# RokLenarcic/AhoCorasick

Measured on AMD Instinct MI355X. Metric: haystack MB/s (UTF-16 bytes scanned per second, records delivered in reference order), higher is better.
Workload: dtype u16; 1 GPU; BASELINE config 2: AhoCorasickMap, 10k keywords (len 4-12, a-z), 2^29 UTF-16 units (1 GiB at 29); keywords=10000, states=58221, classes=27, table=dense u16, lds_states=2408, units_per_gpu=536870912, matches_per_gpu=1332068, matches_total=1332068, record_bytes=12, parallelism=single, reserve_cus=0

## Files before the change

ahocorasick_amd/csrc/acgpu_kernels.hip:

```cpp
#include <hip/hip_runtime.h>

#include <algorithm>
#include <type_traits>
#include <utility>

#include "acgpu_device.h"
#include "acgpu_forms.h"

namespace acgpu {

#ifndef ACGPU_SCAN_MINBLOCKS
#define ACGPU_SCAN_MINBLOCKS 1
#endif
#ifndef ACGPU_DFA_CHAINS
#define ACGPU_DFA_CHAINS 2
#endif
constexpr int kScanBlock = 1024;
constexpr int kQueueCap = 128;
constexpr int kQueueFlush = kQueueCap - kWave;

int scan_block_threads() { return kScanBlock; }
size_t scan_queue_bytes(int block_threads) { return (size_t)(block_threads / kWave) * kQueueCap * sizeof(ScratchRec); }

struct WaveQueue {
// ... 765 lines not shown
    return hipGetLastError();
}


struct TokenTables {
    const uint16_t *kw_units;
    const uint32_t *kw_off;
    uint32_t n_kw;
    const uint16_t *swapcase;
    const uint16_t *script_units;
    uint32_t script_off[7];
    uint16_t seps[6];
};
__device__ __forceinline__ uint64_t synth_draw(uint64_t seed, uint64_t idx) {
    uint64_t x = seed + (idx + 1) * 0x9E3779B97F4A7C15ull;
    uint64_t z = (x ^ (x >> 30)) * 0xBF58476D1CE4E5B9ull;
    z = (z ^ (z >> 27)) * 0x94D049BB133111EBull;
    return z ^ (z >> 31);
}
__device__ __forceinline__ uint32_t synth_bounded(uint64_t z, uint32_t k) { return (uint32_t)(((z >> 32) * (uint64_t)k) >> 32); }

__global__ __launch_bounds__(256) void k_token_lengths(TokenTables T, uint64_t seed, uint32_t n_tokens, uint32_t *len) {
    const uint32_t t = blockIdx.x * blockDim.x + threadIdx.x;
    if (t >= n_tokens) return;
    const uint64_t d0 = (uint64_t)t * 32;
    uint32_t wl;
    if (synth_bounded(synth_draw(seed, d0), 2) == 0 && T.n_kw) {
        const uint32_t wi = synth_bounded(synth_draw(seed, d0 + 1), T.n_kw);
        wl = T.kw_off[wi + 1] - T.kw_off[wi];
    } else {
        wl = 2 + synth_bounded(synth_draw(seed, d0 + 2), 11);
    }
    len[t] = wl + 1 + synth_bounded(synth_draw(seed, d0 + 28), 3);
}

__global__ __launch_bounds__(256) void k_token_fill(TokenTables T, uint64_t seed, uint32_t n_tokens, const uint64_t *start, uint16_t *dst,
                                                    uint64_t n_units) {
    const uint32_t t = blockIdx.x * blockDim.x + threadIdx.x;
    if (t >= n_tokens) return;
    uint64_t at = start[t];
    if (at >= n_units) return;
    const uint64_t d0 = (uint64_t)t * 32;
    auto put = [&](uint32_t u) {
        if (at < n_units) dst[at] = (uint16_t)u;
        ++at;
    };
    if (synth_bounded(synth_draw(seed, d0), 2) == 0 && T.n_kw) {
        const uint32_t wi = synth_bounded(synth_draw(seed, d0 + 1), T.n_kw);
        const uint32_t a = T.kw_off[wi], wl = T.kw_off[wi + 1] - a;
        for (uint32_t i = 0; i < wl; ++i) {
            uint32_t u = T.kw_units[a + i];
            if (T.swapcase && i < 24 && synth_bounded(synth_draw(seed, d0 + 2 + i), 2)) u = T.swapcase[u];
            put(u);
        }
    } else {
        const uint32_t sc = synth_bounded(synth_draw(seed, d0 + 1), 6);
        const uint32_t wl = 2 + synth_bounded(synth_draw(seed, d0 + 2), 11);
        const uint32_t a = T.script_off[sc], tl = T.script_off[sc + 1] - a;
        for (uint32_t i = 0; i < wl; ++i) put(T.script_units[a + synth_bounded(synth_draw(seed, d0 + 3 + i), tl)]);
    }
    const uint32_t ns = 1 + synth_bounded(synth_draw(seed, d0 + 28), 3);
    for (uint32_t i = 0; i < ns; ++i) put(T.seps[synth_bounded(synth_draw(seed, d0 + 29 + i), 6)]);
}

hipError_t launch_token_stream(uint16_t *d_dst, uint64_t n_units, uint64_t seed, const uint16_t *d_kw_units, const uint32_t *d_kw_off,
                               uint32_t n_kw, const uint16_t *d_swapcase, const uint16_t *d_script_units, const uint32_t *script_off,
                               const uint16_t *seps, uint32_t n_tokens, uint32_t *d_len, uint64_t *d_start, uint64_t *d_tmp,
                               hipStream_t stream) {
    TokenTables T;
    T.kw_units = d_kw_units; T.kw_off = d_kw_off; T.n_kw = n_kw; T.swapcase = d_swapcase; T.script_units = d_script_units;
    for (int i = 0; i < 7; ++i) T.script_off[i] = script_off[i];
    for (int i = 0; i < 6; ++i) T.seps[i] = seps[i];
    const dim3 grid((n_tokens + 255) / 256), block(256);
    hipLaunchKernelGGL(k_token_lengths, grid, block, 0, stream, T, seed, n_tokens, d_len);
    hipError_t e = hipGetLastError();
    if (e != hipSuccess) return e;
    e = launch_exclusive_scan(d_len, n_tokens, d_start, d_tmp, stream);
    if (e != hipSuccess) return e;
    hipLaunchKernelGGL(k_token_fill, grid, block, 0, stream, T, seed, n_tokens, d_start, d_dst, n_units);
    return hipGetLastError();
}

__global__ __launch_bounds__(1024) void k_stream_probe(const uint4 *__restrict__ p, uint64_t n_tiles, unsigned *sink) {
    const uint32_t lane = threadIdx.x & 63u;
    const uint64_t wave = (uint64_t)blockIdx.x * (blockDim.x / 64) + threadIdx.x / 64;
    const uint64_t n_waves = (uint64_t)gridDim.x * (blockDim.x / 64);
    const uint64_t per_wave = (n_tiles + n_waves - 1) / n_waves;
    const uint64_t t0 = wave * per_wave, t1 = t0 + per_wave < n_tiles ? t0 + per_wave : n_tiles;
    if (t0 >= t1) return;
    uint32_t x = 0;
    uint4 cur[4], nxt[4];
    const uint4 *b = p + t0 * 256 + lane * 4;
#pragma unroll
    for (int u = 0; u < 4; ++u) nxt[u] = b[u];
    for (uint64_t t = t0; t < t1; ++t) {
#pragma unroll
        for (int u = 0; u < 4; ++u) cur[u] = nxt[u];
        const uint4 *nb = p + (t + 1 < t1 ? t + 1 : t) * 256 + lane * 4;
#pragma unroll
        for (int u = 0; u < 4; ++u) nxt[u] = nb[u];
#pragma unroll
        for (int u = 0; u < 4; ++u) x ^= cur[u].x ^ cur[u].y ^ cur[u].z ^ cur[u].w;
    }
    if (x == 0x12345678u) sink[0] = x;
}

__global__ __launch_bounds__(256) void k_stream_probe_best(const uint4 *__restrict__ p, uint64_t n_groups, unsigned *sink) {
    const uint32_t lane = threadIdx.x & 63u;
    const uint64_t wave = (uint64_t)blockIdx.x * (blockDim.x / 64) + threadIdx.x / 64;
    const uint64_t n_waves = (uint64_t)gridDim.x * (blockDim.x / 64);
    uint32_t x = 0;
    for (uint64_t g = wave; g < n_groups; g += n_waves) {
        uint4 buf[4][2];
#pragma unroll
        for (int d = 0; d < 4; ++d) {
            const uint4 *b = p + (g * 4 + d) * 128;
            buf[d][0] = b[lane * 2];
            buf[d][1] = b[lane * 2 + 1];
        }
#pragma unroll
        for (int d = 0; d < 4; ++d) x ^= buf[d][0].x ^ buf[d][0].y ^ buf[d][0].z ^ buf[d][0].w ^ buf[d][1].x ^ buf[d][1].y ^ buf[d][1].z ^ buf[d][1].w;
    }
    if (x == 0x12345678u) sink[0] = x;
}

hipError_t launch_stream_probe(const void *d_buf, uint64_t n_bytes, int n_cu, unsigned *d_sink, int pattern, hipStream_t stream) {
    if (pattern == 1) {
        const uint64_t n_groups = n_bytes / 8192;
        if (n_groups == 0) return hipErrorInvalidValue;
        hipLaunchKernelGGL(k_stream_probe_best, dim3(n_cu * 8), dim3(256), 0, stream, reinterpret_cast<const uint4 *>(d_buf), n_groups, d_sink);
        return hipGetLastError();
    }
    const uint64_t n_tiles = n_bytes / 4096;
    if (n_tiles == 0) return hipErrorInvalidValue;
    hipLaunchKernelGGL(k_stream_probe, dim3(n_cu), dim3(1024), 0, stream, reinterpret_cast<const uint4 *>(d_buf), n_tiles, d_sink);
    return hipGetLastError();
}

}
```

ahocorasick_amd/csrc/acgpu_tile.hip:

```cpp
#include <hip/hip_runtime.h>

#include <utility>

#include "acgpu_tile_common.h"

namespace acgpu {

int tile_block_threads() { return kTileBlock; }
uint32_t tile_reserve_slots() { return kReserve; }
uint32_t tile_group_units() { return kPrefetch * kTileUnits; }

#ifndef ACGPU_FILTER_WORDS
#define ACGPU_FILTER_WORDS 22016
#endif
constexpr int kFilterWordsMax = ACGPU_FILTER_WORDS;

static_assert(kVerifyBatches * kWave + 128 <= kL2Cap, "the queue holds what a drain leaves plus a tile's survivors (-DACGPU_NB=4 hangs)");
constexpr int kBigFresh = 704;
static_assert(kBigFresh * 2 * (kTileBlock / kWave) <= kL2Words * 4, "the lists of the large second level live where the Bloom words did");

struct __attribute__((packed, aligned(2))) Units8 {
    uint32_t d[4];
};

struct Vec16 {
    unsigned long long lo, hi;
};
__device__ __forceinline__ Vec16 stream_load(const uint16_t *hay, uint32_t unit) {
    const unsigned char *p = reinterpret_cast<const unsigned char *>(hay) + (size_t)(unit * 2u);
    typedef unsigned long long v2ul __attribute__((ext_vector_type(2)));
#ifdef ACGPU_STREAM_NT
    const v2ul v = __builtin_nontemporal_load(reinterpret_cast<const v2ul *>(p));
#else
    const v2ul v = *reinterpret_cast<const v2ul *>(p);
#endif
    return Vec16{v.x, v.y};
}

template <bool RANGE>
__device__ __forceinline__ uint32_t tile_class_t(const DevTables &T, uint32_t unit) {
    if (RANGE) return min(unit - T.cls_base, T.cls_span);
    if (T.hashk && T.fold_range) {
        if (unit & T.fr_himask) return T.tile_lut[unit];
        return min(min(min(unit - T.fr_base, unit - T.fr_base2), min(unit - T.fr_base3, unit - T.fr_base4)), T.fr_span);
    }
    return T.tile_lut[unit];
}

__device__ __forceinline__ uint32_t rchild(const DevTables &T, uint32_t id, uint32_t unit, uint32_t cls) {
    if (T.rdense) return T.rtab[id * T.filt_n + cls];
    const uint32_t u = T.cs ? unit : (uint32_t)T.lower[unit];
    const uint32_t r = hashed_goto(T.rhkeys, T.rhvals, T.rhmask, id, u);
    return r == ~0u ? 0u : r;
}

template <bool RANGE>
__device__ __forceinline__ uint32_t walk_step(const DevTables &T, uint32_t ref, uint32_t unit) {
    const uint32_t cls = tile_class_t<RANGE>(T, unit);
    const uint32_t hint = (ref >> kRefHintShift) & kRefHintMask;
    if (hint != 0 && hint - 1 != cls) return 0;
    return rchild(T, ref & kRefIdMask, unit, cls);
}

template <int K, bool RANGE, bool HASHK = false, bool QI = false, bool SHORTS = true>
__device__ __forceinline__ void verify_multi(TileCtx &c, uint32_t head, uint32_t n_cand) {
    constexpr int NB = kVerifyBatches;
    const DevTables &T = *c.Tp;
    const TileLaunch &L = *c.Lp;
    const uint16_t *hay = L.d_hay;
    const uint32_t lane = lane_id();
    bool act[NB];
    uint32_t e[NB], ref[NB], ref0[NB], child0[NB], left_unit[NB], d[NB], m[NB], one_len[NB], one_node[NB], info[NB], lcls[NB];
    Units8 win[NB];
#pragma unroll
    for (int b = 0; b < NB; ++b) {
        const uint32_t q = b * kWave + lane;
        act[b] = q < n_cand;
        if (QI) {
            e[b] = act[b] ? c.pos_base + (uint32_t)c.pos16[head + q] + 1 : 8;
            info[b] = act[b] ? c.cand[head + q] : 0u;
        } else {
            e[b] = act[b] ? c.cand[head + q] + 1 : 8;
            info[b] = 0;
        }
        m[b] = 0; one_len[b] = 0; one_node[b] = 0; d[b] = K; left_unit[b] = 0;
    }
    uint32_t kidx[NB];
    bool need_win = true;
    if (QI) {
        bool unknown = false;
#pragma unroll
        for (int b = 0; b < NB; ++b) unknown |= act[b] && !(info[b] & kQiKnown);
        need_win = __any(unknown);
    }
#ifdef ACGPU_TIMING
    unsigned long long vt0 = clock64();
#define VT_MARK(i) { asm volatile("s_waitcnt vmcnt(0)" ::: "memory"); const unsigned long long t_ = clock64(); c.vt[i] += t_ - vt0; vt0 = t_; }
#else
#define VT_MARK(i)
#endif
#pragma unroll
    for (int b = 0; b < NB; ++b) {
        if (!need_win) {
            win[b] = Units8{{0, 0, 0, 0}};
        } else if (e[b] >= 8) {
            if (ACGPU_DBG(L, 8u)) win[b] = Units8{{e[b], e[b] * 3u, e[b] * 5u, e[b] * 7u}};
            else win[b] = *reinterpret_cast<const Units8 *>(hay + e[b] - 8);
        } else {
            win[b] = Units8{{0, 0, 0, 0}};
#pragma unroll
            for (int j = 0; j < 8; ++j) {
                if (e[b] + j >= 8) win[b].d[j >> 1] |= (uint32_t)hay[e[b] + j - 8] << (16 * (j & 1));
            }
        }
    }
    VT_MARK(0)
#pragma unroll
    for (int b = 0; b < NB; ++b) {
        uint32_t idx = 0;
// ... 334 lines not shown
__global__ __launch_bounds__(kTileBlock) void k_ac_tile(DevTables T, TileLaunch L) {
    static_assert(!BIG || L2, "the large second level is a form of the L2 kernel");
#ifdef ACGPU_TIMING
    const unsigned long long tm_entry = clock64();
    unsigned long long tm_startup = 0;
#endif
    const bool has_short = SHORTS && T.has_short != 0;
    __shared__ __attribute__((aligned(16))) uint32_t rows32[SPLIT ? kFilterWordsSplit : (L2 ? kFilterWordsL2 : kFilterWordsMax)];
    extern __shared__ __attribute__((aligned(16))) unsigned char smem[];
    __shared__ uint32_t wg_words[kFtWords];
    const bool FT = !SPLIT && L.fused_tail != 0;
    const unsigned char *rows8 = reinterpret_cast<const unsigned char *>(rows32);
    uint32_t *cand_all = reinterpret_cast<uint32_t *>(smem);
    constexpr uint32_t kRowsPer = (sizeof(rows32) / 16 + kTileBlock - 1) / kTileBlock;
    constexpr uint32_t kBloomPer = (L2 && !BIG) ? (kL2Words / 4 + kTileBlock - 1) / kTileBlock : 0u;
    const uint32_t n4 = T.filt_words / 4;
    const uint4 *src4 = reinterpret_cast<const uint4 *>(T.filt_bits);
    uint4 tab[kRowsPer + kBloomPer];
#pragma unroll
    for (uint32_t q = 0; q < kRowsPer; ++q) {
        const uint32_t i = threadIdx.x + q * blockDim.x;
        tab[q] = make_uint4(0u, 0u, 0u, 0u);
        if (i < n4) tab[q] = src4[i];
    }
#pragma unroll
    for (uint32_t q = 0; q < kBloomPer; ++q) {
        const uint32_t i = threadIdx.x + q * blockDim.x;
        tab[kRowsPer + q] = reinterpret_cast<const uint4 *>(T.l2_bloom)[min(i, (uint32_t)kL2Words / 4 - 1)];
    }
    if (FT) {
        if (threadIdx.x == 0) ft_take_number(L, wg_words);
        __syncthreads();
    }
    const uint32_t pg_off = (T.filt_words * 4u + 15u) & ~15u;
    const bool cls_lds = !RANGE && !PK && T.cls_pages != nullptr && (uint64_t)pg_off + T.cls_pages_bytes <= sizeof(rows32) && !ACGPU_DBG(L, 1u << 15);
    const unsigned char *pg8 = rows8 + pg_off;
    constexpr int D2 = K + 2 < 6 ? K + 2 : 6;
    constexpr int kAcVec = L2 ? kL2Vec : acgpu::kAcVec;
    constexpr int kAcLaneUnits = 8 * kAcVec;
    constexpr int kAcTileUnits = kWave * kAcLaneUnits;
    constexpr int kAcTiles = kPrefetch / kAcVec;
    static_assert(kAcTiles >= 1 && kAcLaneUnits <= 32, "tile geometry");
    constexpr int kAcCandCap = kAcTileUnits + kVerifyBatches * kWave;
    constexpr uint32_t kQueueCap = L2 ? kL2Cap : kAcCandCap;
    const uint32_t wave_in_block = __builtin_amdgcn_readfirstlane(threadIdx.x / kWave);
    constexpr int kWavesPerBlock = kTileBlock / kWave;
    uint16_t *pos16_all = reinterpret_cast<uint16_t *>(smem + kWavesPerBlock * kL2Cap * 4);
    unsigned char *tb = smem + kWavesPerBlock * kL2Cap * 6 + wave_in_block * kTbBytes;
    uint16_t *fresh = reinterpret_cast<uint16_t *>(smem + kWavesPerBlock * (kL2Cap * 6 + kTbBytes)) + wave_in_block * kL2Fresh;
    uint32_t *bloom = reinterpret_cast<uint32_t *>(smem + (kTileBlock / kWave) * kL2WaveBytes);
    uint16_t *bigl = reinterpret_cast<uint16_t *>(bloom) + wave_in_block * kBigFresh;
    static_assert(kL2Words % 4 == 0, "Bloom words are copied 16 bytes at a time");

    const uint32_t lane = lane_id();
    const uint32_t wg = FT ? __builtin_amdgcn_readfirstlane(wg_words[0]) : blockIdx.x;
    const uint32_t wave_global = wg * (kTileBlock / kWave) + wave_in_block;
    TileCtx c{&T, &L, SPLIT ? L.d_cands + (size_t)wave_global * L.cands_per_wave : cand_all + wave_in_block * kQueueCap, 0, 0, 0u, 0};
    c.wg = wg;
    if (L2) c.pos16 = pos16_all + wave_in_block * kL2Cap;
    uint32_t lane0 = 0;
    const uint32_t slice_base = SPLIT ? wave_global * L.cands_per_wave : 0u;
    uint32_t region_first = 0;

    constexpr uint32_t ROWB = WIDE ? 8 : 4;
    const uint32_t n = T.filt_n;
    uint32_t nK1s = ROWB;
#pragma unroll
    for (int i = 0; i < K - 1; ++i) nK1s *= n;
    const int neg_nK1s = -(int)nK1s;
    constexpr int NP = L2 ? D2 / 2 : K / 2;

    const uint32_t first_region = wave_global * L.regions_per_wave;
    const bool has_work = first_region < L.n_regions;
    const uint32_t last_region = min(first_region + L.regions_per_wave, L.n_regions);
    const uint32_t base8 = L.own_begin & ~7u;
    const uint32_t R = L.region_units;
    const uint32_t span_begin = max(L.own_begin, base8 + first_region * R);
    uint32_t span_end = base8 + last_region * R;
    if (span_end > L.own_end || last_region == L.n_regions) span_end = L.own_end;
    const uint32_t nfull = L.n_units & ~7u;
    const uint32_t hi = min(span_end, nfull);
    const uint32_t last_vec = nfull >= 8 ? nfull - 8 : 0;
    const uint16_t *hay = L.d_hay;

    uint32_t wave_total = 0;
    uint32_t region = first_region;
    uint32_t boundary = base8 + (region + 1) * R;
    uint32_t rb = span_begin;
    uint32_t re = min(span_end, boundary);
    c.pos_base = boundary - R;
    uint32_t tile = base8 + first_region * R;

    bool vec_todo = has_work && tile < hi;
    bool tail_todo = has_work && span_end > nfull;
    uint32_t d0 = 0;
    uint32_t prio_turn = 0;
    bool mid = false;
    uint32_t carry[4] = {0, 0, 0, 0};
    Vec16 nxt[kAcTiles][kAcVec], grp[kAcTiles][kAcVec];
#pragma unroll
    for (int d = 0; d < kAcTiles; ++d)
#pragma unroll
        for (int u = 0; u < kAcVec; ++u) nxt[d][u] = grp[d][u] = Vec16{0ull, 0ull};
    if (vec_todo) {
        if (K > 1 && tile >= 8) {
            const uint4 p = *reinterpret_cast<const uint4 *>(hay + tile - 8);
            carry[0] = p.x; carry[1] = p.y; carry[2] = p.z; carry[3] = p.w;
        }
#pragma unroll
        for (int d = 0; d < kAcTiles; ++d)
#pragma unroll
            for (int u = 0; u < kAcVec; ++u)
                nxt[d][u] = stream_load(hay, min(tile + d * kAcTileUnits + lane * kAcLaneUnits + u * 8, last_vec));
    }
    {
        uint4 *dst4 = reinterpret_cast<uint4 *>(rows32);
#pragma unroll
        for (uint32_t q = 0; q < kRowsPer; ++q) {
            const uint32_t i = threadIdx.x + q * blockDim.x;
            if (i < n4) dst4[i] = tab[q];
        }
        for (uint32_t i = threadIdx.x + kRowsPer * blockDim.x; i < n4; i += blockDim.x) dst4[i] = src4[i];
        for (uint32_t i = n4 * 4 + threadIdx.x; i < T.filt_words; i += blockDim.x) rows32[i] = T.filt_bits[i];
#pragma unroll
        for (uint32_t q = 0; q < kBloomPer; ++q) {
            const uint32_t i = threadIdx.x + q * blockDim.x;
            if (i < (uint32_t)kL2Words / 4) reinterpret_cast<uint4 *>(bloom)[i] = tab[kRowsPer + q];
        }
        if (L2 && !BIG)
            for (uint32_t i = threadIdx.x + kBloomPer * blockDim.x; i < (uint32_t)kL2Words / 4; i += blockDim.x)
                reinterpret_cast<uint4 *>(bloom)[i] = reinterpret_cast<const uint4 *>(T.l2_bloom)[i];
        if (cls_lds)
            for (uint32_t i = threadIdx.x; i < T.cls_pages_bytes / 16; i += blockDim.x)
                reinterpret_cast<uint4 *>(rows32)[pg_off / 16 + i] = reinterpret_cast<const uint4 *>(T.cls_pages)[i];
    }
    __syncthreads();
    if (!has_work && !FT) return;

#ifdef ACGPU_TIMING
    unsigned long long tm[8] = {0, 0, 0, 0, 0, 0, 0, 0};
    const unsigned long long tm_start = clock64();
#define TM_BEGIN const unsigned long long tm_t0 = clock64()
#define TM_END(i) tm[i] += clock64() - tm_t0
#else
#define TM_BEGIN
#define TM_END(i)
#endif
    for (;;) {
        const bool seam = vec_todo ? (!mid && tile >= boundary) : true;
        const uint32_t keep = SPLIT ? ~0u : (seam ? 1u : (uint32_t)(kVerifyBatches * kWave));
        if (vec_todo && !mid) {
#ifndef ACGPU_NO_SETPRIO
            switch ((wave_in_block / 4u + prio_turn++) & 3u) {
            case 0: __builtin_amdgcn_s_setprio(0); break;
            case 1: __builtin_amdgcn_s_setprio(1); break;
            case 2: __builtin_amdgcn_s_setprio(2); break;
            default: __builtin_amdgcn_s_setprio(3); break;
            }
#endif
#ifdef ACGPU_TIMING
            { TM_BEGIN; asm volatile("s_waitcnt vmcnt(0)" ::: "memory"); TM_END(1); tm[4]++; }
#endif
#pragma unroll
            for (int d = 0; d < kAcTiles; ++d)
#pragma unroll
                for (int u = 0; u < kAcVec; ++u) grp[d][u] = nxt[d][u];
        }
        if (!SPLIT && c.cand_n >= keep && c.cand_n != 0) {
            TM_BEGIN;
            drain<K, RANGE, HASHK, L2, SHORTS>(c, keep);
            TM_END(2);
#ifdef ACGPU_TIMING
            tm[5]++;
#endif
        }

        if (vec_todo) {
            if (!mid) {
                if (tile >= boundary) {
                    if (SPLIT) {
                        if (lane == 0) L.d_region_cands[region] = make_uint2(slice_base + region_first, c.cand_n - region_first);
                        region_first = c.cand_n;
                    } else if (lane == 0 && !FT) {
                        L.d_region_counts[region] = c.rank_base;
                    }
                    if (!FT) {
                        wave_total += c.rank_base;
                        c.rank_base = 0;
                    }
                    ++region;
                    rb = boundary;
                    c.pos_base = boundary;
                    boundary += R;
                    re = min(span_end, boundary);
                }
#pragma unroll
                for (int d = 0; d < kAcTiles; ++d)
#pragma unroll
                    for (int u = 0; u < kAcVec; ++u)
                        nxt[d][u] = stream_load(hay, min(tile + (kAcTiles + d) * kAcTileUnits + lane * kAcLaneUnits + u * 8, last_vec));
            }
#ifdef ACGPU_TIMING
            const unsigned long long tm_f0 = clock64();
            if (tm_startup == 0) tm_startup = tm_f0 - tm_entry;
#endif
            const uint32_t lo = has_short ? rb : max(rb, (uint32_t)(K - 1));
            const uint32_t top = min(re, hi);
            const bool edge = tile < lo || tile + kAcTiles * kAcTileUnits > top;
            bool resume = false;
#pragma unroll
            for (int d = 0; d < kAcTiles; ++d) {
                if ((uint32_t)d < d0) continue;
                const uint32_t cur = tile + d * kAcTileUnits;
                if (cur >= hi) break;
                if (SPLIT) {
                    if (c.cand_n + kAcTileUnits > L.cands_per_wave) {
                        if (lane == 0) atomicOr(L.d_overflow, 1u);
                        return;
                    }
                } else if (!L2 && c.cand_n > kAcCandCap - kAcTileUnits) {
                    d0 = d;
                    resume = true;
                    break;
                }
                uint32_t carry_in[4];
#pragma unroll
                for (int q = 0; q < 4; ++q) carry_in[q] = carry[q];
                const uint32_t v = cur + lane * kAcLaneUnits;
                uint32_t ww[4 * kAcVec];
#pragma unroll
                for (int u = 0; u < kAcVec; ++u) {
                    ww[4 * u + 0] = (uint32_t)grp[d][u].lo; ww[4 * u + 1] = (uint32_t)(grp[d][u].lo >> 32);
                    ww[4 * u + 2] = (uint32_t)grp[d][u].hi; ww[4 * u + 3] = (uint32_t)(grp[d][u].hi >> 32);
                }
                uint32_t pp[4] = {0, 0, 0, 0};
#pragma unroll
                for (int q = 4 - NP; q < 4; ++q) {
                    const uint32_t mine = ww[4 * (kAcVec - 1) + q];
                    pp[q] = from_prev_lane(mine, carry[q]);
                    carry[q] = __builtin_amdgcn_readlane(mine, 63);
                }
                uint32_t mask = 0;
                if (ACGPU_DBG(L, 4u)) {
                    uint32_t x = 0;
#pragma unroll
                    for (int q = 0; q < 4 * kAcVec; ++q) x ^= ww[q];
                    mask = (x == 0x12345678u) ? 1u : 0u;
                } else if (PK) {
                    constexpr int ND = 4 + 4 * kAcVec;
                    const uint32_t base2 = (RANGE ? T.cls_base : T.fr_base) * 0x10001u, span2 = (RANGE ? T.cls_span : T.fr_span) * 0x10001u;
                    const uint32_t baseB2 = T.fr_base2 * 0x10001u, n2 = n * 0x10001u;
                    const uint32_t baseC2 = T.fr_base3 * 0x10001u, baseD2 = T.fr_base4 * 0x10001u;
                    bool by_table = false;
                    if (!RANGE && T.fr_himask != 0) {
                        uint32_t any_bits = 0;
#pragma unroll
                        for (int D = 4 - NP; D < 4; ++D) any_bits |= pp[D];
#pragma unroll
                        for (int q = 0; q < 4 * kAcVec; ++q) any_bits |= ww[q];
                        by_table = __any((any_bits & (T.fr_himask * 0x10001u)) != 0);
                    }
                    auto classes_of = [&](uint32_t units2) -> uint32_t {
                        if (RANGE) return pk_class(units2, base2, span2);
                        if (by_table) return (uint32_t)T.tile_lut[units2 & 0xffffu] | ((uint32_t)T.tile_lut[units2 >> 16] << 16);
                        const uint32_t c1 = pk_class(units2, base2, span2), c2 = pk_class(units2, baseB2, span2);
                        if (!NR4) return pk_min(c1, c2);
                        const uint32_t c3 = pk_class(units2, baseC2, span2), c4 = pk_class(units2, baseD2, span2);
                        return pk_min(pk_min(c1, c2), pk_min(c3, c4));
                    };
                    uint32_t CC[ND], MM[ND], B8[ND / 2];
#pragma unroll
                    for (int D = 4 - NP; D < 4; ++D) CC[D] = classes_of(pp[D]);
#pragma unroll
                    for (int D = 4 - NP + 1; D < 4; ++D) MM[D] = __builtin_amdgcn_alignbit(CC[D], CC[D - 1], 16);
                    if (L2) {
#pragma unroll
                        for (int i = 0; i < 2; ++i)
                            B8[i] = (2 * i + 1 >= 4 - NP) ? __builtin_amdgcn_perm(CC[2 * i + 1], 2 * i >= 4 - NP ? CC[2 * i] : 0u, 0x06040200u) : 0u;
                        if (lane == 0) *reinterpret_cast<uint2 *>(tb + 8) = make_uint2(B8[0], B8[1]);
                    }
                    uint32_t acc = 0;
#pragma unroll
                    for (int u = 0; u < kAcVec; ++u) {
#pragma unroll
                        for (int D = 4 + 4 * u; D < 8 + 4 * u; ++D) {
                            CC[D] = classes_of(ww[D - 4]);
                            MM[D] = __builtin_amdgcn_alignbit(CC[D], CC[D - 1], 16);
                        }
#pragma unroll
                        for (int D = 4 + 4 * u; D < 8 + 4 * u; ++D) {
                            const int S0 = 2 * D - (K - 1);
                            uint32_t H = (S0 & 1) ? MM[(S0 + 1) / 2] : CC[S0 / 2];
#pragma unroll
                            for (int t = 1; t < K - 1; ++t) {
                                const int S = S0 + t;
                                H = pk_mad(H, n2, (S & 1) ? MM[(S + 1) / 2] : CC[S / 2]);
                            }
                            const uint32_t row_lo = rows32[ACGPU_DBG(L, 8192u) ? ((H & 0xffe0u) | (lane & 31u)) : (H & 0xffffu)];
                            const uint32_t row_hi = rows32[ACGPU_DBG(L, 8192u) ? (((H >> 16) & 0xffe0u) | (lane & 31u)) : (H >> 16)];
                            acc = __builtin_amdgcn_alignbit(row_lo >> (CC[D] & 31u), acc, 1);
                            acc = __builtin_amdgcn_alignbit(row_hi >> ((CC[D] >> 16) & 31u), acc, 1);
                        }
                        if (L2) {
                            B8[2 + 2 * u] = __builtin_amdgcn_perm(CC[5 + 4 * u], CC[4 + 4 * u], 0x06040200u);
                            B8[3 + 2 * u] = __builtin_amdgcn_perm(CC[7 + 4 * u], CC[6 + 4 * u], 0x06040200u);
                            if (u & 1)
                                reinterpret_cast<uint4 *>(tb + 16 + lane * kAcLaneUnits)[u / 2] =
                                    make_uint4(B8[2 * u], B8[2 * u + 1], B8[2 * u + 2], B8[2 * u + 3]);
                        }
                        __builtin_amdgcn_sched_barrier(0);
                    }
                    mask = kAcLaneUnits == 32 ? acc : acc >> ((32 - kAcLaneUnits) & 31);
                    if (edge) {
                        asm volatile("" ::: "memory");
                        const uint32_t first = lo > v ? min(lo - v, (uint32_t)kAcLaneUnits) : 0u;
                        const uint32_t last = top > v ? min(top - v, (uint32_t)kAcLaneUnits) : 0u;
                        mask &= (uint32_t)((1ull << last) - 1ull) & ~(uint32_t)((1ull << first) - 1ull);
                    }
                } else {
                    uint32_t a[kAcLaneUnits + K - 1];
                    if (!RANGE && cls_lds) {
                        auto cls_of = [&](uint32_t unit) -> uint32_t { return pg8[256u + ((uint32_t)pg8[unit >> 8] << 8) + (unit & 255u)]; };
#pragma unroll
                        for (int j = 0; j < K - 1; ++j) {
                            const int u = 8 - (K - 1) + j;
                            a[j] = cls_of((pp[u >> 1] >> (16 * (u & 1))) & 0xffffu);
                        }
#pragma unroll
                        for (int j = 0; j < kAcLaneUnits; ++j) a[K - 1 + j] = cls_of((ww[j >> 1] >> (16 * (j & 1))) & 0xffffu);
                    } else {
#pragma unroll
                    for (int j = 0; j < K - 1; ++j) {
                        const int u = 8 - (K - 1) + j;
                        a[j] = tile_class_t<RANGE>(T, (pp[u >> 1] >> (16 * (u & 1))) & 0xffffu);
                    }
#pragma unroll
                    for (int j = 0; j < kAcLaneUnits; ++j)
                        a[K - 1 + j] = tile_class_t<RANGE>(T, (ww[j >> 1] >> (16 * (j & 1))) & 0xffffu);
                    }
                    uint32_t hs = 0;
#pragma unroll
                    for (int j = 0; j < K - 1; ++j) hs = __umul24(hs, n) + a[j] * ROWB;
#pragma unroll
                    for (int j = 0; j < kAcLaneUnits; ++j) {
                        if (j > 0 && K > 1) hs = roll_row<ROWB>(hs, n, a[j - 1], neg_nK1s, a[j + K - 2]);
                        uint32_t bit;
                        if (WIDE) {
                            const uint64_t row = *reinterpret_cast<const uint64_t *>(rows8 + hs);
                            bit = (uint32_t)(row >> a[K - 1 + j]) & 1u;
                        } else {
                            const uint32_t row = *reinterpret_cast<const uint32_t *>(rows8 + hs);
                            bit = __builtin_amdgcn_ubfe(row, a[K - 1 + j], 1);
                        }
                        mask |= bit << j;
                    }
                    if (edge) {
                        const uint32_t first = lo > v ? min(lo - v, (uint32_t)kAcLaneUnits) : 0u;
                        const uint32_t last = top > v ? min(top - v, (uint32_t)kAcLaneUnits) : 0u;
                        mask &= ((1u << last) - 1u) & ~((1u << first) - 1u);
                    }
                }
                if (ACGPU_DBG(L, 512u)) mask &= 0x0101u << (lane & 7u);
                if (!L2) {
                    enqueue(c, mask, v);
                    continue;
                }
                if (lane < lane0) mask = 0;
                uint32_t cnt = __popc(mask);
                uint32_t incl = wave_inclusive_scan_dpp(cnt);
                uint32_t total = __builtin_amdgcn_readlane(incl, kWave - 1);
                if (total == 0) {
                    lane0 = 0;
                    continue;
                }
                struct __attribute__((packed, aligned(1), may_alias)) Win8b { uint32_t lo, hi; };
                if (BIG && total <= (uint32_t)kBigFresh) {
                    {
                        uint32_t slot = incl - cnt, m = mask;
                        while (__any(m != 0)) {
                            if (m != 0) {
                                bigl[slot++] = (uint16_t)(lane * kAcLaneUnits + (uint32_t)__builtin_ctz(m));
                                m &= m - 1;
                            }
                        }
                    }
                    __builtin_amdgcn_wave_barrier();
                    const unsigned char *tb8 = tb + 16;
                    const uint32_t *bigtab = T.l2_big;
                    uint32_t survivors = 0;
                    for (uint32_t b = 0; b < total; b += 4u * kWave) {
                        uint32_t word[4], hh[4], pp[4];
#pragma unroll
                        for (int q = 0; q < 4; ++q) {
                            const uint32_t k = b + (uint32_t)q * kWave + lane;
                            pp[q] = k < total ? (uint32_t)bigl[k] : 0u;
                            const Win8b w = *reinterpret_cast<const Win8b *>(tb8 + (int)pp[q] - 7);
                            const uint32_t cl[4] = {w.hi >> 24, (w.hi >> 16) & 0xffu, (w.hi >> 8) & 0xffu, w.hi & 0xffu};
                            hh[q] = l2_hash(K == 4 ? w.hi : l2_gram(cl, K));
                            word[q] = bigtab[l2_word_big(hh[q])];
                        }
#pragma unroll
                        for (int q = 0; q < 4; ++q) {
                            const uint32_t k = b + (uint32_t)q * kWave + lane;
                            const bool act = k < total;
                            const Win8b w = *reinterpret_cast<const Win8b *>(tb8 + (int)pp[q] - 7);
                            const uint32_t cls[6] = {w.hi >> 24, (w.hi >> 16) & 0xffu, (w.hi >> 8) & 0xffu, w.hi & 0xffu, w.lo >> 24, (w.lo >> 16) & 0xffu};
                            const uint32_t pat = l2_pattern(hh[q]);
                            bool pass = false;
#pragma unroll
                            for (int len = K; len <= D2; ++len) {
                                const uint32_t bits = __builtin_amdgcn_alignbit(pat, pat, l2_rot(cls, len, K));
                                pass |= (word[q] & bits) == bits;
                            }
                            if (has_short) {
                                uint32_t hrow = T.filt_other;
#pragma unroll
                                for (int j = K - 2; j >= 1; --j) hrow = hrow * n + cls[j];
                                pass = pass || ((rows32[hrow] >> cls[0]) & 1u);
                            }
                            pass = pass && act;
                            if (act) bigl[k] = (uint16_t)(pp[q] | (pass ? 0x8000u : 0u));
                            survivors += (uint32_t)__popcll(__ballot(pass));
                        }
                    }
                    __builtin_amdgcn_wave_barrier();
                    if (survivors <= 128u && c.cand_n + survivors <= (uint32_t)kL2Cap) {
                        for (uint32_t b = 0; b < total; b += kWave) {
                            const uint32_t k = b + lane;
                            const uint32_t e = k < total ? (uint32_t)bigl[k] : 0u;
                            const bool pass = (e & 0x8000u) != 0;
                            const uint32_t p = e & 0x7fffu;
                            const uint64_t bal = __ballot(pass);
                            if (bal == 0) continue;
                            if (pass) {
                                const Win8b w = *reinterpret_cast<const Win8b *>(tb8 + (int)p - 7);
                                const uint32_t cls[6] = {w.hi >> 24, (w.hi >> 16) & 0xffu, (w.hi >> 8) & 0xffu, w.hi & 0xffu, w.lo >> 24, (w.lo >> 16) & 0xffu};
                                uint32_t shortbit = 0;
                                if (has_short) {
                                    uint32_t hrow = T.filt_other;
#pragma unroll
                                    for (int j = K - 2; j >= 1; --j) hrow = hrow * n + cls[j];
                                    shortbit = (rows32[hrow] >> cls[0]) & 1u;
                                }
                                const uint32_t at = c.cand_n + (uint32_t)__popcll(bal & lanemask_lt());
                                uint32_t idx = cls[K - 1];
#pragma unroll
                                for (int j = K - 2; j >= 0; --j) idx = __umul24(idx, n) + cls[j];
                                c.pos16[at] = (uint16_t)(cur + p - c.pos_base);
                                c.cand[at] = HASHK ? (kQiChecked | (shortbit ? kQiShort : 0u)) : kQiKnown | kQiChecked | (shortbit ? kQiShort : 0u) | (cls[K] << kQiLeftShift) | idx;
                            }
                            c.cand_n += (uint32_t)__popcll(bal);
                        }
                        __builtin_amdgcn_wave_barrier();
                        lane0 = 0;
                        continue;
                    }
                    {
                        uint32_t keep = 0;
                        for (uint32_t j = 0; j < cnt; ++j) {
                            const uint32_t e = bigl[incl - cnt + j];
                            if (e & 0x8000u) keep |= 1u << ((e & 0x7fffu) - lane * kAcLaneUnits);
                        }
                        __builtin_amdgcn_wave_barrier();
                        mask = keep;
                        cnt = __popc(mask);
                        incl = wave_inclusive_scan_dpp(cnt);
                        total = __builtin_amdgcn_readlane(incl, kWave - 1);
                    }
                }
                if (!BIG && total <= (uint32_t)kL2Fresh && c.cand_n + total <= (uint32_t)kL2Cap) {
                    uint32_t slot = incl - cnt, m = mask;
                    while (__any(m != 0)) {
                        if (m != 0) {
                            fresh[slot++] = (uint16_t)(lane * kAcLaneUnits + (uint32_t)__builtin_ctz(m));
                            m &= m - 1;
                        }
                    }
                    __builtin_amdgcn_wave_barrier();
                    struct __attribute__((packed, aligned(1), may_alias)) Win8 { uint32_t lo, hi; };
                    const unsigned char *tb8 = tb + 16;
                    for (uint32_t b = 0; b < total; b += kWave) {
                        const uint32_t k = b + lane;
                        const bool act = k < total;
                        const uint32_t p = act ? (uint32_t)fresh[k] : 0u;
                        const Win8 w = *reinterpret_cast<const Win8 *>(tb8 + (int)p - 7);
                        const uint32_t cls[6] = {w.hi >> 24, (w.hi >> 16) & 0xffu, (w.hi >> 8) & 0xffu, w.hi & 0xffu, w.lo >> 24, (w.lo >> 16) & 0xffu};
                        const uint32_t h = l2_hash(K == 4 ? w.hi : l2_gram(cls, K));
                        const uint32_t word = bloom[l2_word(h)];
                        const uint32_t pat = l2_pattern(h);
                        bool pass = false;
#pragma unroll
                        for (int len = K; len <= D2; ++len) {
                            const uint32_t bits = __builtin_amdgcn_alignbit(pat, pat, l2_rot(cls, len, K));
                            pass |= (word & bits) == bits;
                        }
                        uint32_t shortbit = 0;
                        if (has_short) {
                            uint32_t hrow = T.filt_other;
#pragma unroll
                            for (int j = K - 2; j >= 1; --j) hrow = hrow * n + cls[j];
                            shortbit = (rows32[hrow] >> cls[0]) & 1u;
                        }
                        pass = (pass || shortbit || ACGPU_DBG(L, 4096u)) && act;
                        const uint64_t bal = __ballot(pass);
                        if (pass) {
                            const uint32_t at = c.cand_n + (uint32_t)__popcll(bal & lanemask_lt());
                            uint32_t idx = cls[K - 1];
#pragma unroll
#ifdef ACGPU_PK_C
                            for (int j = K - 2; j >= 0; --j) idx = __umul24(idx, n) + cls[j];
#else
                            for (int j = K - 2; j >= 0; --j) asm("v_mad_u32_u24 %0, %1, %2, %3" : "=v"(idx) : "v"(idx), "s"(n), "v"(cls[j]));
#endif
                            c.pos16[at] = (uint16_t)(cur + p - c.pos_base);
                            c.cand[at] = HASHK ? (kQiChecked | (shortbit ? kQiShort : 0u)) : kQiKnown | kQiChecked | (shortbit ? kQiShort : 0u) | (cls[K] << kQiLeftShift) | idx;
                        }
                        c.cand_n += (uint32_t)__popcll(bal);
                    }
                    __builtin_amdgcn_wave_barrier();
                    lane0 = 0;
                    continue;
                }
                if (c.cand_n >= (uint32_t)(kVerifyBatches * kWave)) {
#pragma unroll
                    for (int q = 0; q < 4; ++q) carry[q] = carry_in[q];
                    d0 = d;
                    resume = true;
                    break;
                }
                {
                    const uint32_t room = (uint32_t)kL2Cap - c.cand_n;
                    const uint32_t nl = (uint32_t)__popcll(__ballot(incl <= room));
                    uint32_t slot = c.cand_n + incl - cnt, m = lane < nl ? mask : 0u;
                    while (__any(m != 0)) {
                        if (m != 0) {
                            c.pos16[slot] = (uint16_t)(v + (uint32_t)__builtin_ctz(m) - c.pos_base);
                            c.cand[slot++] = 0u;
                            m &= m - 1;
                        }
                    }
                    c.cand_n += __builtin_amdgcn_readlane(incl, nl - 1);
                    __builtin_amdgcn_wave_barrier();
                    if (nl < (uint32_t)kWave) {
                        lane0 = nl;
#pragma unroll
                        for (int q = 0; q < 4; ++q) carry[q] = carry_in[q];
                        d0 = d;
                        resume = true;
                        break;
                    }
                    lane0 = 0;
                }
            }
#ifdef ACGPU_TIMING
            tm[3] += clock64() - tm_f0;
#endif
            mid = resume;
            if (!resume) {
                d0 = 0;
                tile += kAcTiles * kAcTileUnits;
                vec_todo = tile < hi;
            }
            continue;
        }
        if (tail_todo) {
            tail_todo = false;
            const uint32_t t0 = max(nfull, span_begin);
            if (t0 >= boundary) {
                if (SPLIT) {
                    if (lane == 0) L.d_region_cands[region] = make_uint2(slice_base + region_first, c.cand_n - region_first);
                    region_first = c.cand_n;
                } else if (lane == 0 && !FT) {
                    L.d_region_counts[region] = c.rank_base;
                }
                if (!FT) {
                    wave_total += c.rank_base;
                    c.rank_base = 0;
                }
                ++region;
                c.pos_base = boundary;
            }
            if (SPLIT && c.cand_n + kWave > L.cands_per_wave) {
                if (lane == 0) atomicOr(L.d_overflow, 1u);
                return;
            }
            const uint32_t pos = t0 + lane;
            uint32_t mask = 0;
            if (pos < span_end && (pos + 1 >= (uint32_t)K || has_short) && !ACGPU_DBG(L, 4u)) {
                uint32_t hrow = 0;
                for (int j = K - 1; j >= 1; --j) hrow = hrow * n + (pos >= (uint32_t)j ? tile_class_t<RANGE>(T, hay[pos - j]) : T.filt_other);
                const uint32_t last = tile_class_t<RANGE>(T, hay[pos]);
                const uint32_t word = rows32[hrow * (ROWB / 4) + (last >> 5)];
                mask = (word >> (last & 31)) & 1u;
            }
            if (L2) {
                const uint64_t bal = __ballot(mask != 0);
                if (mask != 0) {
                    const uint32_t at = c.cand_n + (uint32_t)__popcll(bal & lanemask_lt());
                    c.pos16[at] = (uint16_t)(pos - c.pos_base);
                    c.cand[at] = 0u;
                }
                c.cand_n += (uint32_t)__popcll(bal);
                __builtin_amdgcn_wave_barrier();
            } else {
                enqueue(c, mask, pos);
            }
            continue;
        }
        break;
    }
    if (SPLIT) {
        if (lane == 0) L.d_region_cands[region] = make_uint2(slice_base + region_first, c.cand_n - region_first);
        return;
    }
#ifdef ACGPU_TIMING
    tm[0] = clock64() - tm_start;
    if (lane == 0 && L.d_timing)
    {
        for (int i = 0; i < 8; ++i) L.d_timing[(size_t)wave_global * 8 + i] = tm[i];
        L.d_timing[(size_t)wave_global * 8 + 4] = tm[4] | (tm_startup << 32);
        L.d_timing[(size_t)wave_global * 8 + 6] = c.vt[0] | (c.vt[1] << 32);
        L.d_timing[(size_t)wave_global * 8 + 7] = c.vt[2] | (c.vt[3] << 32);
    }
#endif
    if (lane == 0 && has_work && !FT) L.d_region_counts[region] = c.rank_base;
    wave_total += c.rank_base;
    if (lane == 0 && L.wg_sums && wave_total) atomicAdd(L.d_counter + (size_t)wg * kCounterStride + 1, (unsigned long long)wave_total);
    if (FT) {
        tile_fused_tail(L, wg, wg_words, wave_total, c.res_cur, c.res_left, c.slot_limit);
// ... 73 lines not shown
```

Baseline: 4.127 million MB/s.

## Stream haystack through buffer loads into a single register set, reloading in place

The scan kernel drops the separate nxt/grp double buffer and reads the haystack with raw buffer loads that use per-lane offsets and a scalar group offset. Each vector is reloaded as soon as its classes have been computed, so there is one register set instead of two and no copy per group. Resume after a mid-group stall now reuses a saved mask instead of restoring the carries. This cuts VGPR pressure and address arithmetic but adds waitcnt ordering and redo-path complexity that could break correctness or stall on memory latency. The stream probe kernel is also converted to buffer loads.

Measured after the change: 3.511 million MB/s. -14.9%, worse.

```diff
diff --git a/ahocorasick_amd/csrc/acgpu_kernels.hip b/ahocorasick_amd/csrc/acgpu_kernels.hip
--- a/ahocorasick_amd/csrc/acgpu_kernels.hip
+++ b/ahocorasick_amd/csrc/acgpu_kernels.hip
@@ -871,25 +871,29 @@
 }
 
 __global__ __launch_bounds__(1024) void k_stream_probe(const uint4 *__restrict__ p, uint64_t n_tiles, unsigned *sink) {
+    typedef uint32_t v4u __attribute__((ext_vector_type(4)));
     const uint32_t lane = threadIdx.x & 63u;
-    const uint64_t wave = (uint64_t)blockIdx.x * (blockDim.x / 64) + threadIdx.x / 64;
+    const uint64_t wave = (uint64_t)blockIdx.x * (blockDim.x / 64) + __builtin_amdgcn_readfirstlane(threadIdx.x / 64);
     const uint64_t n_waves = (uint64_t)gridDim.x * (blockDim.x / 64);
     const uint64_t per_wave = (n_tiles + n_waves - 1) / n_waves;
     const uint64_t t0 = wave * per_wave, t1 = t0 + per_wave < n_tiles ? t0 + per_wave : n_tiles;
-    if (t0 >= t1) return;
-    uint32_t x = 0;
-    uint4 cur[4], nxt[4];
-    const uint4 *b = p + t0 * 256 + lane * 4;
-#pragma unroll
-    for (int u = 0; u < 4; ++u) nxt[u] = b[u];
-    for (uint64_t t = t0; t < t1; ++t) {
-#pragma unroll
-        for (int u = 0; u < 4; ++u) cur[u] = nxt[u];
-        const uint4 *nb = p + (t + 1 < t1 ? t + 1 : t) * 256 + lane * 4;
-#pragma unroll
-        for (int u = 0; u < 4; ++u) nxt[u] = nb[u];
-#pragma unroll
-        for (int u = 0; u < 4; ++u) x ^= cur[u].x ^ cur[u].y ^ cur[u].z ^ cur[u].w;
+    if (t0 >= t1 || (t1 - t0) * 4096 > 0xffffffffull) return;
+    const uint32_t tiles = (uint32_t)(t1 - t0);
+    const __amdgpu_buffer_rsrc_t rs = __builtin_amdgcn_make_buffer_rsrc(const_cast<uint4 *>(p + t0 * 256), 0, (int)(tiles * 4096u), 0x00020000);
+    uint32_t x = 0, off[4];
+    v4u v[4];
+#pragma unroll
+    for (int u = 0; u < 4; ++u) {
+        off[u] = lane * 64 + u * 16;
+        v[u] = __builtin_amdgcn_raw_buffer_load_b128(rs, (int)off[u], 0, 0);
+    }
+    for (uint32_t t = 0; t < tiles; ++t) {
+        const uint32_t next = (t + 1 < tiles ? t + 1 : t) * 4096u;
+#pragma unroll
+        for (int u = 0; u < 4; ++u) {
+            x ^= v[u].x ^ v[u].y ^ v[u].z ^ v[u].w;
+            v[u] = __builtin_amdgcn_raw_buffer_load_b128(rs, (int)off[u], (int)next, 0);
+        }
     }
     if (x == 0x12345678u) sink[0] = x;
 }
diff --git a/ahocorasick_amd/csrc/acgpu_tile.hip b/ahocorasick_amd/csrc/acgpu_tile.hip
--- a/ahocorasick_amd/csrc/acgpu_tile.hip
+++ b/ahocorasick_amd/csrc/acgpu_tile.hip
@@ -23,18 +23,16 @@
     uint32_t d[4];
 };
 
-struct Vec16 {
-    unsigned long long lo, hi;
-};
-__device__ __forceinline__ Vec16 stream_load(const uint16_t *hay, uint32_t unit) {
-    const unsigned char *p = reinterpret_cast<const unsigned char *>(hay) + (size_t)(unit * 2u);
-    typedef unsigned long long v2ul __attribute__((ext_vector_type(2)));
+typedef uint32_t Vec16 __attribute__((ext_vector_type(4)));
+__device__ __forceinline__ __amdgpu_buffer_rsrc_t stream_rsrc(const uint16_t *hay, uint32_t nfull) {
+    return __builtin_amdgcn_make_buffer_rsrc(const_cast<uint16_t *>(hay), 0, (int)(nfull * 2u), 0x00020000);
+}
+__device__ __forceinline__ Vec16 stream_load(__amdgpu_buffer_rsrc_t rs, uint32_t lane_bytes, uint32_t tile_bytes) {
 #ifdef ACGPU_STREAM_NT
-    const v2ul v = __builtin_nontemporal_load(reinterpret_cast<const v2ul *>(p));
+    return __builtin_amdgcn_raw_buffer_load_b128(rs, (int)lane_bytes, (int)tile_bytes, 2);
 #else
-    const v2ul v = *reinterpret_cast<const v2ul *>(p);
-#endif
-    return Vec16{v.x, v.y};
+    return __builtin_amdgcn_raw_buffer_load_b128(rs, (int)lane_bytes, (int)tile_bytes, 0);
+#endif
 }
 
 template <bool RANGE>
@@ -535,6 +533,17 @@
     const uint32_t hi = min(span_end, nfull);
     const uint32_t last_vec = nfull >= 8 ? nfull - 8 : 0;
     const uint16_t *hay = L.d_hay;
+    constexpr uint32_t kGroupUnits = kAcTiles * kAcTileUnits;
+    const uint32_t last_vec_bytes = __builtin_amdgcn_readfirstlane(last_vec * 2u);
+    uint32_t lane_off[kAcTiles][kAcVec], group_off = 0;
+    auto set_stream_offsets = [&](uint32_t g) {
+        group_off = min(g * 2u, last_vec_bytes);
+        const uint32_t left = last_vec_bytes - group_off;
+#pragma unroll
+        for (int d = 0; d < kAcTiles; ++d)
+#pragma unroll
+            for (int u = 0; u < kAcVec; ++u) lane_off[d][u] = min((d * kAcTileUnits + lane * kAcLaneUnits) * 2 + u * 16, left);
+    };
 
     uint32_t wave_total = 0;
     uint32_t region = first_region;
@@ -549,22 +558,23 @@
     uint32_t d0 = 0;
     uint32_t prio_turn = 0;
     bool mid = false;
+    uint32_t saved_mask = 0;
     uint32_t carry[4] = {0, 0, 0, 0};
-    Vec16 nxt[kAcTiles][kAcVec], grp[kAcTiles][kAcVec];
+    Vec16 grp[kAcTiles][kAcVec];
 #pragma unroll
     for (int d = 0; d < kAcTiles; ++d)
 #pragma unroll
-        for (int u = 0; u < kAcVec; ++u) nxt[d][u] = grp[d][u] = Vec16{0ull, 0ull};
+        for (int u = 0; u < kAcVec; ++u) grp[d][u] = Vec16{0u, 0u, 0u, 0u};
     if (vec_todo) {
         if (K > 1 && tile >= 8) {
             const uint4 p = *reinterpret_cast<const uint4 *>(hay + tile - 8);
             carry[0] = p.x; carry[1] = p.y; carry[2] = p.z; carry[3] = p.w;
         }
+        set_stream_offsets(tile);
 #pragma unroll
         for (int d = 0; d < kAcTiles; ++d)
 #pragma unroll
-            for (int u = 0; u < kAcVec; ++u)
-                nxt[d][u] = stream_load(hay, min(tile + d * kAcTileUnits + lane * kAcLaneUnits + u * 8, last_vec));
+            for (int u = 0; u < kAcVec; ++u) grp[d][u] = stream_load(stream_rsrc(hay, nfull), lane_off[d][u], group_off);
     }
     {
         uint4 *dst4 = reinterpret_cast<uint4 *>(rows32);
@@ -614,10 +624,6 @@
 #ifdef ACGPU_TIMING
             { TM_BEGIN; asm volatile("s_waitcnt vmcnt(0)" ::: "memory"); TM_END(1); tm[4]++; }
 #endif
-#pragma unroll
-            for (int d = 0; d < kAcTiles; ++d)
-#pragma unroll
-                for (int u = 0; u < kAcVec; ++u) grp[d][u] = nxt[d][u];
         }
         if (!SPLIT && c.cand_n >= keep && c.cand_n != 0) {
             TM_BEGIN;
@@ -647,11 +653,8 @@
                     boundary += R;
                     re = min(span_end, boundary);
                 }
-#pragma unroll
-                for (int d = 0; d < kAcTiles; ++d)
-#pragma unroll
-                    for (int u = 0; u < kAcVec; ++u)
-                        nxt[d][u] = stream_load(hay, min(tile + (kAcTiles + d) * kAcTileUnits + lane * kAcLaneUnits + u * 8, last_vec));
+                group_off = (tile + kGroupUnits) * 2u;
+                if (tile + 2 * kGroupUnits > nfull) set_stream_offsets(tile + kGroupUnits);
             }
 #ifdef ACGPU_TIMING
             const unsigned long long tm_f0 = clock64();
@@ -676,29 +679,38 @@
                     resume = true;
                     break;
                 }
-                uint32_t carry_in[4];
-#pragma unroll
-                for (int q = 0; q < 4; ++q) carry_in[q] = carry[q];
+                const bool redo = L2 && mid && (uint32_t)d == d0;
+                __builtin_amdgcn_s_waitcnt(0x0f70);
                 const uint32_t v = cur + lane * kAcLaneUnits;
                 uint32_t ww[4 * kAcVec];
 #pragma unroll
-                for (int u = 0; u < kAcVec; ++u) {
-                    ww[4 * u + 0] = (uint32_t)grp[d][u].lo; ww[4 * u + 1] = (uint32_t)(grp[d][u].lo >> 32);
-                    ww[4 * u + 2] = (uint32_t)grp[d][u].hi; ww[4 * u + 3] = (uint32_t)(grp[d][u].hi >> 32);
-                }
+                for (int u = 0; u < kAcVec; ++u)
+#pragma unroll
+                    for (int q = 0; q < 4; ++q) ww[4 * u + q] = grp[d][u][q];
+                auto reload = [&](int u, uint32_t after0, uint32_t after1) {
+                    const uint16_t *base = hay;
+                    asm volatile("" : "+s"(group_off), "+s"(base) : "v"(after0), "v"(after1));
+                    grp[d][u] = stream_load(stream_rsrc(base, nfull), lane_off[d][u], group_off);
+                };
                 uint32_t pp[4] = {0, 0, 0, 0};
-#pragma unroll
-                for (int q = 4 - NP; q < 4; ++q) {
-                    const uint32_t mine = ww[4 * (kAcVec - 1) + q];
-                    pp[q] = from_prev_lane(mine, carry[q]);
-                    carry[q] = __builtin_amdgcn_readlane(mine, 63);
+                if (!redo) {
+#pragma unroll
+                    for (int q = 4 - NP; q < 4; ++q) {
+                        const uint32_t mine = ww[4 * (kAcVec - 1) + q];
+                        pp[q] = from_prev_lane(mine, carry[q]);
+                        carry[q] = __builtin_amdgcn_readlane(mine, 63);
+                    }
                 }
                 uint32_t mask = 0;
-                if (ACGPU_DBG(L, 4u)) {
+                if (redo) {
+                    mask = saved_mask;
+                } else if (ACGPU_DBG(L, 4u)) {
                     uint32_t x = 0;
 #pragma unroll
                     for (int q = 0; q < 4 * kAcVec; ++q) x ^= ww[q];
                     mask = (x == 0x12345678u) ? 1u : 0u;
+#pragma unroll
+                    for (int u = 0; u < kAcVec; ++u) reload(u, x, x);
                 } else if (PK) {
                     constexpr int ND = 4 + 4 * kAcVec;
                     const uint32_t base2 = (RANGE ? T.cls_base : T.fr_base) * 0x10001u, span2 = (RANGE ? T.cls_span : T.fr_span) * 0x10001u;
@@ -740,6 +752,7 @@
                             CC[D] = classes_of(ww[D - 4]);
                             MM[D] = __builtin_amdgcn_alignbit(CC[D], CC[D - 1], 16);
                         }
+                        reload(u, MM[5 + 4 * u], MM[7 + 4 * u]);
 #pragma unroll
                         for (int D = 4 + 4 * u; D < 8 + 4 * u; ++D) {
                             const int S0 = 2 * D - (K - 1);
@@ -791,6 +804,8 @@
                     for (int j = 0; j < kAcLaneUnits; ++j)
                         a[K - 1 + j] = tile_class_t<RANGE>(T, (ww[j >> 1] >> (16 * (j & 1))) & 0xffffu);
                     }
+#pragma unroll
+                    for (int u = 0; u < kAcVec; ++u) reload(u, a[K - 1 + 8 * u + 3], a[K - 1 + 8 * u + 7]);
                     uint32_t hs = 0;
 #pragma unroll
                     for (int j = 0; j < K - 1; ++j) hs = __umul24(hs, n) + a[j] * ROWB;
@@ -814,6 +829,7 @@
                     }
                 }
                 if (ACGPU_DBG(L, 512u)) mask &= 0x0101u << (lane & 7u);
+                if (L2) saved_mask = mask;
                 if (!L2) {
                     enqueue(c, mask, v);
                     continue;
@@ -915,7 +931,7 @@
                             if (e & 0x8000u) keep |= 1u << ((e & 0x7fffu) - lane * kAcLaneUnits);
                         }
                         __builtin_amdgcn_wave_barrier();
-                        mask = keep;
+                        mask = saved_mask = keep;
                         cnt = __popc(mask);
                         incl = wave_inclusive_scan_dpp(cnt);
                         total = __builtin_amdgcn_readlane(incl, kWave - 1);
@@ -975,8 +991,6 @@
                     continue;
                 }
                 if (c.cand_n >= (uint32_t)(kVerifyBatches * kWave)) {
-#pragma unroll
-                    for (int q = 0; q < 4; ++q) carry[q] = carry_in[q];
                     d0 = d;
                     resume = true;
                     break;
@@ -996,8 +1010,6 @@
                     __builtin_amdgcn_wave_barrier();
                     if (nl < (uint32_t)kWave) {
                         lane0 = nl;
-#pragma unroll
-                        for (int q = 0; q < 4; ++q) carry[q] = carry_in[q];
                         d0 = d;
                         resume = true;
                         break;
```
